# pycompression/python-zlib-ng

Measured on AMD Instinct MI355X. Metric: MB/s compress+decompress, 128 KiB blocks level 6, higher is better.
Workload: dtype u8

## Files before the change

### python-zlib-ng_amd/csrc/za_deflate.hip

```cpp
#include "za_common.h"
#include "za_crc.h"
#include <type_traits>

#define ZA_CH_GROUP 16
#define ZA_CH_OFFS(x) (((x) >> (32 - ZA_HASH_BITS - 2)) & (((1u << ZA_HASH_BITS) - 1u) << 2))
#define ZA_CH_CHUNK (64 * ZA_CH_GROUP)
#if defined(ZA_CH_STATS) || defined(ZA_ABL_CH_NOHASH) || defined(ZA_ABL_CH_NOATOMIC) || defined(ZA_ABL_CH_NOCHECK) || defined(ZA_ABL_CH_NOSTORE) || \
    defined(ZA_ABL_CH_HALFREADS) || defined(ZA_ABL_CH_HALFWRITES)
#undef ZA_CH_PAIR
#define ZA_CH_PAIR 0
#endif
#ifndef ZA_CH_PAIR
#define ZA_CH_PAIR 1
#endif
#ifdef ZA_CH_FORCE_FIX
#define ZA_CH_FORCE_FIX_ON true
#else
#define ZA_CH_FORCE_FIX_ON false
#endif

typedef uint32_t za_v4u32 __attribute__((ext_vector_type(4)));
__device__ __forceinline__ void za_issue_load16(za_v4u32 &dst, const uint8_t *addr)
{
    asm volatile("global_load_dwordx4 %0, %1, off" : "=v"(dst) : "v"(addr) : "memory");
// ... 893 lines not shown
            const uint32_t idx = P & (ZA_BYTES - 1), w = idx >> 2, sh = idx & 3u;
            const uint32_t m0 = win32[w], m1 = win32[w + 1], m2 = win32[w + 2], m3 = win32[w + 3], m4 = win32[w + 4];
            me0 = __builtin_amdgcn_alignbyte(m1, m0, sh); me1 = __builtin_amdgcn_alignbyte(m2, m1, sh);
            me2 = __builtin_amdgcn_alignbyte(m3, m2, sh); me3 = __builtin_amdgcn_alignbyte(m4, m3, sh);
        };
        auto finish = [&](int p, uint32_t P, uint32_t me0, uint32_t me1, uint32_t me2, uint32_t me3, int maxlen, int cap, int nice,
                          int best_len, int best_dist, uint32_t own_b, uint32_t own_c) {
#pragma unroll
            for (int t = 0; t < (USEC ? 2 : 1); t++) {
                const int dl = maxlen >= ZA_MIN_MATCH ? (int)(t == 0 ? own_b : own_c) : 0;
                if (dl != 0 && dl <= L.max_dist && best_len < nice) {
                    const uint32_t q = P - (uint32_t)dl;
                    const uint32_t sh = q & 3u;
                    const uint32_t *cw = (const uint32_t *)(lds + (q & (uint32_t)(ZA_BYTES - 4)));
                    const uint32_t c0 = cw[0], c1 = cw[1], c2 = cw[2], c3 = cw[3], c4 = cw[4];
                    const uint32_t x0 = __builtin_amdgcn_alignbyte(c1, c0, sh) ^ me0, x1 = __builtin_amdgcn_alignbyte(c2, c1, sh) ^ me1;
                    const uint32_t x2 = __builtin_amdgcn_alignbyte(c3, c2, sh) ^ me2, x3 = __builtin_amdgcn_alignbyte(c4, c3, sh) ^ me3;
                    uint32_t fbit, f1, f2, f3;
                    asm("v_ffbl_b32 %0, %4\n\tv_ffbl_b32 %1, %5\n\tv_ffbl_b32 %2, %6\n\tv_ffbl_b32 %3, %7\n\t"
                        "v_add_u32_e64 %1, %1, 32 clamp\n\tv_add_u32_e64 %2, %2, 64 clamp\n\tv_add_u32_e64 %3, %3, %8 clamp\n\t"
                        "v_min3_u32 %0, %0, %1, %2\n\tv_min_u32_e32 %0, %0, %3"
                        : "=&v"(fbit), "=&v"(f1), "=&v"(f2), "=&v"(f3) : "v"(x0), "v"(x1), "v"(x2), "v"(x3), "s"(96u));
                    int len = (int)min(fbit >> 3, 16u);
                    if (len == 16 && cap > 16) len = za_search_extend(win32, q, P, len, maxlen);
                    len = len < cap ? len : cap;
                    const bool better = len > best_len || (len == best_len && dl < best_dist);
                    best_len = better ? len : best_len;
                    best_dist = better ? dl : best_dist;
                }
            }
            uint32_t result = 0;
            if (best_len >= ZA_MIN_MATCH && !(best_len == 3 && best_dist > L.too_far3) && !(best_len == 4 && best_dist > L.too_far4))
                result = ((uint32_t)best_len << 15) | (uint32_t)(best_dist - 1);
            longm = longm || best_len > 64;
            best[p] = __builtin_amdgcn_perm(me0, result, 0x04020100u);
        };
        auto push = [&](bool alive, int p, uint32_t P, uint32_t q, int best_len, int best_dist, int depth) {
            const unsigned long long m = __ballot(alive);
            if (alive) {
                const uint32_t at = wl_n + __builtin_amdgcn_mbcnt_hi((uint32_t)(m >> 32), __builtin_amdgcn_mbcnt_lo((uint32_t)m, 0u));
                wl[2 * at] = (uint32_t)(p - base) | ((uint32_t)best_len << 12) | ((uint32_t)depth << 21);
                wl[2 * at + 1] = (P - q) | ((uint32_t)best_dist << 16);
            }
            wl_n += (uint32_t)__builtin_popcountll(m);
            __builtin_amdgcn_fence(__ATOMIC_RELEASE, "wavefront");
            __builtin_amdgcn_wave_barrier();
        };
        auto batch = [&](uint32_t nb) {
            wl_n -= nb;
            const bool has = (uint32_t)lane < nb;
            uint32_t e0 = 0, e1 = 0;
            __builtin_amdgcn_fence(__ATOMIC_ACQUIRE, "wavefront");
            if (has) { e0 = wl[2 * (wl_n + lane)]; e1 = wl[2 * (wl_n + lane) + 1]; }
            __builtin_amdgcn_fence(__ATOMIC_ACQ_REL, "wavefront");
            __builtin_amdgcn_wave_barrier();
            bool alive = false;
            int p = 0, best_len = 0, best_dist = 0, depth = 0;
            uint32_t P = 0, q = 0;
            if (has) {
                p = base + (int)(e0 & 0xFFFu);
                best_len = (int)((e0 >> 12) & 0x1FFu); depth = (int)(e0 >> 21); best_dist = (int)(e1 >> 16);
                P = goff + (uint32_t)(ZA_WIN + p);
                q = P - (e1 & 0xFFFFu);
                int seg_end = ((p >> sshift) + 1) << sshift;
                if (seg_end > n) seg_end = n;
                int maxlen = seg_end - p;
                if (maxlen > ZA_MAX_MATCH) maxlen = ZA_MAX_MATCH;
                const int cap = L.cap < maxlen ? L.cap : maxlen, nice = L.nice < cap ? L.nice : cap;
                uint32_t me0, me1, me2, me3;
                my16(P, me0, me1, me2, me3);
                const uint32_t sq = q % ZA_RING;
                uint32_t qb = RING_B0 + 2u * sq;
                uint32_t d = *(const uint16_t *)(lds + qb);
                alive = visit(P, me0, me1, me2, me3, maxlen, cap, nice, q, qb, d, best_len, best_dist, depth);
                if (!alive) finish(p, P, me0, me1, me2, me3, maxlen, cap, nice, best_len, best_dist, (uint32_t)linkb[p], USEC ? (uint32_t)linkc[p] : 0u);
            }
            push(alive, p, P, q, best_len, best_dist, depth);
        };
        uint32_t slot = (goff + (uint32_t)(ZA_WIN + base + tid)) % ZA_RING;
        load_own_links(base + ZA_SEARCH_TILE);
#pragma unroll
        for (int k = 0; k < ZA_SEARCH_TILE / ZA_SEARCH_THREADS; k++, slot = slot + ZA_SEARCH_THREADS >= ZA_RING ? slot + ZA_SEARCH_THREADS - ZA_RING : slot + ZA_SEARCH_THREADS) {
            const int p = base + k * ZA_SEARCH_THREADS + tid;
            bool alive = false;
            const uint32_t P = goff + (uint32_t)(ZA_WIN + p);
            uint32_t q = P;
            int best_len = ZA_MIN_MATCH - 1, best_dist = 0, depth = L.chain;
            if (p < n) {
                int seg_end = ((p >> sshift) + 1) << sshift;
                if (seg_end > n) seg_end = n;
                int maxlen = seg_end - p;
                if (maxlen > ZA_MAX_MATCH) maxlen = ZA_MAX_MATCH;
                uint32_t me0, me1, me2, me3;
                my16(P, me0, me1, me2, me3);
                const int cap = L.cap < maxlen ? L.cap : maxlen, nice = L.nice < cap ? L.nice : cap;
                if (maxlen >= ZA_MIN_MATCH) {
                    uint32_t qb = RING_B0 + 2u * slot;
                    uint32_t d = *(const uint16_t *)(lds + qb);
                    alive = visit(P, me0, me1, me2, me3, maxlen, cap, nice, q, qb, d, best_len, best_dist, depth);
                }
                if (!alive) finish(p, P, me0, me1, me2, me3, maxlen, cap, nice, best_len, best_dist, lkb[k], lkc[k]);
            }
            push(alive, p, P, q, best_len, best_dist, depth);
            while (__builtin_amdgcn_readfirstlane((int)wl_n) >= 64) batch(64u);
        }
        for (;;) {
            const uint32_t left = (uint32_t)__builtin_amdgcn_readfirstlane((int)wl_n);
            if (left == 0) break;
            batch(left < 64u ? left : 64u);
        }
        } else {
        uint32_t slot = (goff + (uint32_t)(ZA_WIN + base + (CONSEC ? 4 * tid : tid))) % ZA_RING;
        load_own_links(base + ZA_SEARCH_TILE);
        if (stats && base > 0) stats_issue(base - ZA_SEARCH_TILE);
#ifndef ZA_SEARCH_KUNROLL
#define ZA_SEARCH_KUNROLL 4
#endif
        const int p0c = base + 4 * tid;
        const uint32_t P0c = goff + (uint32_t)(ZA_WIN + p0c);
        uint32_t cm0 = 0, cm1 = 0, cm2 = 0, cm3 = 0, cm4 = 0;
        uint2 cdq = make_uint2(0u, 0u);
        int cseg_end = 0;
        if (CONSEC && p0c < n) {
            const uint32_t w = (P0c & (ZA_BYTES - 1)) >> 2;
            cm0 = win32[w]; cm1 = win32[w + 1]; cm2 = win32[w + 2]; cm3 = win32[w + 3]; cm4 = win32[w + 4];
            cdq = *(const uint2 *)(lds + RING_B0 + 2u * slot);
            cseg_end = ((p0c >> sshift) + 1) << sshift;
            if (cseg_end > n) cseg_end = n;
        }
#pragma unroll
        for (int k = 0; k < ZA_SEARCH_TILE / ZA_SEARCH_THREADS; k++, slot = CONSEC ? slot : slot + ZA_SEARCH_THREADS >= ZA_RING ? slot + ZA_SEARCH_THREADS - ZA_RING : slot + ZA_SEARCH_THREADS) {
            const int p = CONSEC ? p0c + k : base + k * ZA_SEARCH_THREADS + tid;
            res[k] = 0u;
            if (p >= n) continue;
            int seg_end = cseg_end;
            if (!CONSEC) {
                seg_end = ((p >> sshift) + 1) << sshift;
                if (seg_end > n) seg_end = n;
            }
            int maxlen = seg_end - p;
            if (maxlen > ZA_MAX_MATCH) maxlen = ZA_MAX_MATCH;
            uint32_t result = 0;
            const uint32_t P = goff + (uint32_t)(ZA_WIN + p);
            uint32_t me0, me1, me2, me3;
            if (CONSEC) {
                if (k == 0) { me0 = cm0; me1 = cm1; me2 = cm2; me3 = cm3; }
                else {
                    me0 = __builtin_amdgcn_alignbyte(cm1, cm0, (uint32_t)k); me1 = __builtin_amdgcn_alignbyte(cm2, cm1, (uint32_t)k);
                    me2 = __builtin_amdgcn_alignbyte(cm3, cm2, (uint32_t)k); me3 = __builtin_amdgcn_alignbyte(cm4, cm3, (uint32_t)k);
                }
            } else {
                const uint32_t idx = P & (ZA_BYTES - 1), w = idx >> 2, sh = idx & 3u;
                const uint32_t m0 = win32[w], m1 = win32[w + 1], m2 = win32[w + 2], m3 = win32[w + 3], m4 = win32[w + 4];
                me0 = __builtin_amdgcn_alignbyte(m1, m0, sh); me1 = __builtin_amdgcn_alignbyte(m2, m1, sh);
                me2 = __builtin_amdgcn_alignbyte(m3, m2, sh); me3 = __builtin_amdgcn_alignbyte(m4, m3, sh);
            }
            if (maxlen >= ZA_MIN_MATCH) {
                const int cap = L.cap < maxlen ? L.cap : maxlen;
                const int nice = L.nice < cap ? L.nice : cap;
                int best_len = ZA_MIN_MATCH - 1, best_dist = 0;
                uint32_t q = P;
                uint32_t qb = RING_B0 + 2u * (CONSEC ? slot + (uint32_t)k : slot);
                uint32_t d = CONSEC ? ((k < 2 ? cdq.x : cdq.y) >> (16 * (k & 1))) & 0xFFFFu : (uint32_t)*(const uint16_t *)(lds + qb);
                int depth = STEPS > 0 ? STEPS : L.chain;
#pragma unroll
                while (depth-- > 0) {
                    q -= d;
                    qb -= 2u * d;
                    qb += qb < RING_B0 ? RING_BYTES : 0u;
                    const int dist = (int)(P - q);
                    if (dist > L.max_dist) break;
                    d = *(const uint16_t *)(lds + qb);
                    const uint32_t sh = q & 3u;
                    const uint32_t *cw = (const uint32_t *)(lds + (q & (uint32_t)(ZA_BYTES - 4)));
                    const uint32_t c0 = cw[0], c1 = cw[1], c2 = cw[2], c3 = cw[3], c4 = cw[4];
                    uint32_t x0 = __builtin_amdgcn_alignbyte(c1, c0, sh) ^ me0;
                    uint32_t x1 = __builtin_amdgcn_alignbyte(c2, c1, sh) ^ me1;
                    uint32_t x2 = __builtin_amdgcn_alignbyte(c3, c2, sh) ^ me2;
                    uint32_t x3 = __builtin_amdgcn_alignbyte(c4, c3, sh) ^ me3;
                    uint32_t fbit, f1, f2, f3;
                    asm("v_ffbl_b32 %0, %4\n\tv_ffbl_b32 %1, %5\n\tv_ffbl_b32 %2, %6\n\tv_ffbl_b32 %3, %7\n\t"
                        "v_add_u32_e64 %1, %1, 32 clamp\n\tv_add_u32_e64 %2, %2, 64 clamp\n\tv_add_u32_e64 %3, %3, %8 clamp\n\t"
                        "v_min3_u32 %0, %0, %1, %2\n\tv_min_u32_e32 %0, %0, %3"
                        : "=&v"(fbit), "=&v"(f1), "=&v"(f2), "=&v"(f3) : "v"(x0), "v"(x1), "v"(x2), "v"(x3), "s"(96u));
                    int len = (int)min(fbit >> 3, FULL ? 16u : (uint32_t)cap);
                    if (FULL && len == 16 && cap > 16 && best_len < cap &&
                        (best_len < 16 || (uint8_t)za_lds_ld32(win32, q + (uint32_t)best_len) == (uint8_t)za_lds_ld32(win32, P + (uint32_t)best_len))) {
                        len = za_search_extend(win32, q, P, len, maxlen);
                    }
                    if (FULL) len = len < cap ? len : cap;
                    const bool better = len > best_len;
                    best_len = better ? len : best_len;
                    best_dist = better ? dist : best_dist;
                    if (best_len >= nice) break;
                }
                bool from_bc = false;
#ifndef ZA_ABL_SEARCH_NO_B
                {
                    const uint32_t dl = lkb[k];
#ifdef ZA_ABL_BC_SELF
                    const uint32_t q2 = P - (dl & 3u);
#else
                    const uint32_t q2 = P - dl;
#endif
                    const uint32_t *cw = (const uint32_t *)(lds + (q2 & (uint32_t)(ZA_BYTES - 4)));
                    const uint32_t c0 = cw[0], c1 = cw[1];
                    const uint32_t x = (__builtin_amdgcn_alignbyte(c1, c0, q2 & 3u) ^ me0) << 8;
                    const bool better = x == 0u && dl != 0u && (int)dl <= L.max_dist &&
                                        (ZA_HASH_BYTES_B > best_len || (ZA_HASH_BYTES_B == best_len && (int)dl < best_dist));
                    best_len = better ? ZA_HASH_BYTES_B : best_len;
                    best_dist = better ? (int)dl : best_dist;
                    from_bc = better;
                }
#endif
#ifndef ZA_ABL_SEARCH_NO_C
                if (USEC) {
                    const uint32_t dl = lkc[k];
#ifdef ZA_ABL_BC_SELF
                    const uint32_t q2 = P - (dl & 3u);
#else
                    const uint32_t q2 = P - dl;
#endif
                    const uint32_t sh = q2 & 3u;
                    const uint32_t *cw = (const uint32_t *)(lds + (q2 & (uint32_t)(ZA_BYTES - 4)));
                    const uint32_t c0 = cw[0], c1 = cw[1], c2 = cw[2], c3 = cw[3];
                    const uint32_t x = (__builtin_amdgcn_alignbyte(c1, c0, sh) ^ me0) | (__builtin_amdgcn_alignbyte(c2, c1, sh) ^ me1) |
                                       (__builtin_amdgcn_alignbyte(c3, c2, sh) ^ me2);
                    const bool better = x == 0u && dl != 0u && (int)dl <= L.max_dist && cap >= ZA_HASH_BYTES_C &&
                                        (ZA_HASH_BYTES_C > best_len || (ZA_HASH_BYTES_C == best_len && (int)dl < best_dist));
                    best_len = better ? ZA_HASH_BYTES_C : best_len;
                    best_dist = better ? (int)dl : best_dist;
                    from_bc = from_bc || better;
                }
#endif
#ifndef ZA_ABL_NO_EXTEND
                if (!FULL && (best_len == cap || from_bc) && best_len < maxlen) {
                    best_len = za_search_extend(win32, P - (uint32_t)best_dist, P, best_len, maxlen);
                }
#endif
                if (best_len >= ZA_MIN_MATCH && !(best_len == 3 && best_dist > L.too_far3) && !(best_len == 4 && best_dist > L.too_far4))
                    result = ((uint32_t)best_len << 15) | (uint32_t)(best_dist - 1);
                longm = longm || best_len > 64;
            }
#ifdef ZA_ABL_SEARCH_NOLIT
            res[k] = result;
#else
            res[k] = __builtin_amdgcn_perm(me0, result, 0x04020100u);
#endif
        }
        res_base = base;
        }
        if (pq < need_links) store_quad(pq, need_links, nq);
        {
            const int p = bytes_loaded + 8 * tid;
            if (p < need_bytes) {
                const uint64_t v = nbv >> nsh;
                store_bytes(p, (uint32_t)v);
                if (p + 4 < need_bytes) store_bytes(p + 4, (uint32_t)(v >> 32));
            }
        }
        if (ZA_OWN_STAGE) own_store(base + ZA_SEARCH_TILE);
        links_loaded = need_links; bytes_loaded = need_bytes;
        if (stats) { flush_results(); stats_use(); __syncthreads(); }
        else za_lds_barrier();
    }
    if constexpr (!FULL) flush_results();
    if (stats && n > 0) {
        __syncthreads();
        stats_issue((n - 1) & ~(ZA_SEARCH_TILE - 1));
        stats_use();
        for (int d = 32; d >= 1; d >>= 1) { st_U += (uint32_t)__shfl_xor((int)st_U, d, 64); st_NM += (uint32_t)__shfl_xor((int)st_NM, d, 64); }
        if ((tid & 63) == 0) { atomicAdd(&st_cnt[0], st_U); atomicAdd(&st_cnt[1], st_NM); }
        __syncthreads();
        const uint32_t U = st_cnt[0], NM = st_cnt[1];
        uint32_t hh = 0u;
        if (tid < 256) {
            hh = 16u * st_hist[tid] + 1u + (U >> 6);
            st_hist[tid] = 0u;
            uint32_t T = hh;
            for (int d = 32; d >= 1; d >>= 1) T += (uint32_t)__shfl_xor((int)T, d, 64);
            if ((tid & 63) == 0) atomicAdd(&st_cnt[2], T);
        }
        __syncthreads();
        if (tid < 256) {
            const uint32_t T = st_cnt[2];
            uint32_t *cost = cost_ws + (size_t)ui * ZA_DP_COSTS;
            int lbias = za_ilog4(U + NM, U ? U : 1u), mbias = za_ilog4(U + NM, NM ? NM : 1u);
            lbias = lbias > 24 ? 24 : lbias;
            mbias = mbias > 24 ? 24 : mbias;
            const int cl = za_ilog4(T, hh) + lbias;
            cost[tid] = (uint32_t)(cl < 12 ? 12 : cl > 52 ? 52 : cl);
            if (tid == 0) { cost[256] = (uint32_t)(12 + mbias + 20); cost[257] = 0u; }
        }
        __syncthreads();
        if (tid < 4) st_cnt[tid] = 0u;
        st_U = 0u; st_NM = 0u;
    }
    if (L.dp && __ballot(longm) != 0ull && (tid & 63) == 0) cost_ws[(size_t)ui * ZA_DP_COSTS + 258] = 1u;
    carry_bytes = bytes_loaded; n_prev = n;
    }
}

#define ZA_PCH 32
#define ZA_PROW (ZA_PCH + 1)
#ifndef ZA_DP_NEAR
#define ZA_DP_NEAR   64
#endif
#define ZA_DP_ROWS   (ZA_DP_NEAR / 2 + 4)
#ifndef ZA_DCH
#define ZA_DCH       16
#endif
#define ZA_DROW      (ZA_DCH + 1)
#define ZA_DPIECES   (ZA_DCH / 4)
#define ZA_DP_SEGSLOTS 2064

__global__ __launch_bounds__(256) void za_k_dpstats(const ZaUnit *__restrict__ units, const uint32_t *__restrict__ best_ws,
                                                    uint32_t *__restrict__ cost_ws )
{
    __shared__ uint32_t hist[256];
    __shared__ uint32_t cnt[3], tsum;
    const int n = (int)units[blockIdx.x].in_len;
    const int tid = (int)threadIdx.x, lane = tid & 63;
    const uint32_t *best = best_ws + (size_t)blockIdx.x * ZA_BEST_STRIDE;
    hist[tid] = 0;
    if (tid < 3) cnt[tid] = 0;
    if (tid == 0) tsum = 0;
    __syncthreads();
    uint32_t U = 0, NM = 0;
    for (int base = 1024 * (tid >> 6); base < n; base += 4096) {
        const int i0 = base + 4 * lane;
        uint4 v = make_uint4(0u, 0u, 0u, 0u);
        uint32_t pv = 0;
        if (i0 < n) v = *(const uint4 *)(best + i0);
        if (lane == 0 && i0 > 0 && i0 < n) pv = best[i0 - 1];
        const uint32_t e[4] = {v.x, v.y, v.z, v.w};
        uint32_t lp = (uint32_t)__shfl_up((int)ZA_ELEN(v.w), 1, 64);
        if (lane == 0) lp = ZA_ELEN(pv);
#pragma unroll
        for (int k = 0; k < 4; k++) {
            const uint32_t len = ZA_ELEN(e[k]);
            if (i0 + k < n) {
                if (len == 0u || (len == 3u && ZA_EDIST(e[k]) > (uint32_t)ZA_DP_WEAK_DIST)) { atomicAdd(&hist[e[k] >> 24], 1u); U++; }
                else if (len + 1u != lp) NM++;
            }
            lp = len;
        }
    }
    for (int d = 32; d >= 1; d >>= 1) { U += (uint32_t)__shfl_xor((int)U, d, 64); NM += (uint32_t)__shfl_xor((int)NM, d, 64); }
    if (lane == 0) { atomicAdd(&cnt[0], U); atomicAdd(&cnt[1], NM); }
    __syncthreads();
    U = cnt[0]; NM = cnt[1];
    const uint32_t hh = 16u * hist[tid] + 1u + (U >> 6);
    uint32_t T = hh;
    for (int d = 32; d >= 1; d >>= 1) T += (uint32_t)__shfl_xor((int)T, d, 64);
    if (lane == 0) atomicAdd(&tsum, T);
    __syncthreads();
    T = tsum;
    uint32_t *cost = cost_ws + (size_t)blockIdx.x * ZA_DP_COSTS;
    if (n == 0) return;
    int lbias = za_ilog4(U + NM, U ? U : 1u), mbias = za_ilog4(U + NM, NM ? NM : 1u);
    lbias = lbias > 24 ? 24 : lbias;
    mbias = mbias > 24 ? 24 : mbias;
    const int c = za_ilog4(T, hh) + lbias;
    cost[tid] = (uint32_t)(c < 12 ? 12 : c > 52 ? 52 : c);
    if (tid == 0) { cost[256] = (uint32_t)(12 + mbias + 20); cost[257] = 0u; }
}

__device__ __forceinline__ uint32_t za_pk_add_u16(uint32_t a, uint32_t b)
{
    uint32_t r;
    asm("v_pk_add_u16 %0, %1, %2" : "=v"(r) : "v"(a), "v"(b));
    return r;
}

__global__ __launch_bounds__(64) void za_k_optparse(const ZaUnit *__restrict__ units, uint32_t *__restrict__ best_ws,
                                                    const uint32_t *__restrict__ cost_ws, uint32_t *__restrict__ tok_ws ,
                                                    ZaLevel L)
{
    __shared__ uint32_t costt[ZA_DP_COSTS + 4];
    __shared__ uint32_t xt[3 * (ZA_MAX_MATCH + 1)];
    __shared__ uint32_t ring[ZA_DP_ROWS * 64];
    __shared__ uint32_t rowb[64 * ZA_DROW];
#ifndef ZA_DP_PAD
#define ZA_DP_PAD 2304
#endif
#if ZA_DP_PAD > 0
    __shared__ uint32_t dp_pad[ZA_DP_PAD / 4];
    if (units[blockIdx.x].in_len == 0xFFFFFFFFu) {
        dp_pad[threadIdx.x] = blockIdx.x; __syncthreads(); best_ws[threadIdx.x] = dp_pad[(threadIdx.x * 7u + best_ws[0]) % (ZA_DP_PAD / 4)];
    }
#endif
    const ZaUnit u = units[blockIdx.x];
    const int n = (int)u.in_len;
    const int lane = za_lane();
    const int sshift = ZA_UNIT_SEG_SHIFT(u.flags), seg = 1 << sshift;
    const int nseg = (n + seg - 1) >> sshift;
    uint32_t *best = best_ws + (size_t)blockIdx.x * ZA_BEST_STRIDE;
    if (n == 0) return;
    for (int i = lane; i < ZA_DP_COSTS; i += 64) costt[i] = cost_ws[(size_t)blockIdx.x * ZA_DP_COSTS + i];
    if (L.fixed_cost) {
        __syncthreads();
        for (int i = lane; i < 256; i += 64) costt[i] = i < 144 ? 32u : 36u;
        if (lane == 0) costt[256] = 48u;
    }
    for (int len = lane; len <= ZA_MAX_MATCH; len += 64) {
        const int l0 = len > 7 ? len - ZA_DP_SUB : 3;
        uint32_t x[ZA_DP_SUB + 1];
#pragma unroll
        for (int k = 0; k <= ZA_DP_SUB; k++) {
            const int l = l0 + k;
            int lc, ln = 0, le;
            if (l <= ZA_MAX_MATCH) za_len_sym(l, lc, ln, le);
            x[k] = (len >= 3 && l <= len && l >= L.min_len) ? (uint32_t)(4 * ln) : 0x3FFFu;
        }
        xt[3 * len] = x[0] | (x[1] << 16); xt[3 * len + 1] = x[2] | (x[3] << 16); xt[3 * len + 2] = x[4] | ((uint32_t)l0 << 16);
    }
    for (int i = lane; i < ZA_DP_ROWS * 64; i += 64) ring[i] = 0;
    __syncthreads();

    const int s0 = lane << sshift;
    int s1 = s0 + seg;
    if (s1 > n) s1 = n;
    const bool active = lane < nseg;
    uint32_t *myb = rowb + lane * ZA_DROW;
    uint8_t *myring = (uint8_t *)(ring + lane);
    uint16_t *accg = (uint16_t *)(tok_ws + (size_t)blockIdx.x * ZA_TOK_STRIDE) + (size_t)lane * ZA_DP_SEGSLOTS;
    auto ring_put = [&](int slot, uint32_t v) {
        *(uint16_t *)(myring + (slot >> 1) * 256 + (slot & 1) * 2) = (uint16_t)v;
        if (slot < 8) *(uint16_t *)(myring + ((slot >> 1) + ZA_DP_NEAR / 2) * 256 + (slot & 1) * 2) = (uint16_t)v;
    };
    const int mbase = (int)costt[256];
#ifdef ZA_ABL_DP_NOLONG
    const bool has_long = false;
#else
    const bool has_long = costt[258] != 0u;
#endif
    if (active) { ring_put((s1 - s0) & (ZA_DP_NEAR - 1), 0u); accg[s1 - s0] = 0; }
    int acc_next = 0;
    int far_base = -100;
    uint32_t fw[8] = {0u, 0u, 0u, 0u, 0u, 0u, 0u, 0u};
    uint4 pb[ZA_DPIECES];
    auto prefetch = [&](int c) {
#pragma unroll
        for (int j = 0; j < ZA_DPIECES; j++) {
            const int sg = (64 / ZA_DPIECES) * j + lane / ZA_DPIECES, off = (sg << sshift) + c * ZA_DCH + 4 * (lane % ZA_DPIECES);
            pb[j] = make_uint4(0, 0, 0, 0);
            if (c >= 0 && sg < nseg && off < n) pb[j] = *(const uint4 *)(best + off);
        }
    };
    struct Fetch { uint32_t e, clit, x0, x1, x2, w0, w1, w2; };
    auto stage_b = [&](uint32_t e, int idx_p) -> Fetch {
        Fetch f;
        f.e = e;
        f.clit = costt[e >> 24];
        const uint32_t len = ZA_ELEN(e);
        const uint32_t *xr = xt + 3u * len;
        f.x0 = xr[0]; f.x1 = xr[1]; f.x2 = xr[2];
        const uint32_t l0 = len > 7u ? len - (uint32_t)ZA_DP_SUB : 3u;
        const uint32_t st = ((uint32_t)idx_p + l0) & (uint32_t)(ZA_DP_NEAR - 1);
        const uint8_t *rp = myring + (st >> 1) * 256;
        f.w0 = *(const uint32_t *)rp; f.w1 = *(const uint32_t *)(rp + 256); f.w2 = *(const uint32_t *)(rp + 512);
        return f;
    };
    const int nch = ((n < seg ? n : seg) + ZA_DCH - 1) / ZA_DCH;
    uint4 po[ZA_DPIECES];
    uint32_t wacc[ZA_DCH / 2];
    int pend = -1;
    auto flush_pending = [&](auto longs_tag) {
        if (pend < 0) return;
        const int pcb = s0 + pend * ZA_DCH;
        if (decltype(longs_tag)::value && active && pcb < s1) {
            uint4 *g = (uint4 *)(accg + pend * ZA_DCH);
#pragma unroll
            for (int k = 0; k < ZA_DCH / 8; k++) g[k] = make_uint4(wacc[4 * k], wacc[4 * k + 1], wacc[4 * k + 2], wacc[4 * k + 3]);
        }
#pragma unroll
        for (int j = 0; j < ZA_DPIECES; j++) {
            const int sg = (64 / ZA_DPIECES) * j + lane / ZA_DPIECES, off = (sg << sshift) + pend * ZA_DCH + 4 * (lane % ZA_DPIECES);
            if (sg < nseg && off < n) *(uint4 *)(best + off) = po[j];
        }
    };
    prefetch(nch - 1);
    auto walk = [&](auto longs_tag) {
    constexpr bool LONGS = decltype(longs_tag)::value;
#pragma unroll 1
    for (int c = nch - 1; c >= 0; c--) {
        const int cb = s0 + c * ZA_DCH;
        __builtin_amdgcn_wave_barrier();
#pragma unroll
        for (int j = 0; j < ZA_DPIECES; j++) {
            uint32_t *r = rowb + ((64 / ZA_DPIECES) * j + lane / ZA_DPIECES) * ZA_DROW + 4 * (lane % ZA_DPIECES);
            r[0] = pb[j].x; r[1] = pb[j].y; r[2] = pb[j].z; r[3] = pb[j].w;
        }
        __builtin_amdgcn_fence(__ATOMIC_RELEASE, "wavefront");
        __builtin_amdgcn_wave_barrier();
        __builtin_amdgcn_fence(__ATOMIC_ACQUIRE, "wavefront");
        flush_pending(longs_tag);
        prefetch(c - 1);
        if (__ballot(active && cb < s1) != 0ull) {
            const int ib = c * ZA_DCH;
            uint32_t e_a = myb[ZA_DCH - 2];
            Fetch f = stage_b(myb[ZA_DCH - 1], ib + ZA_DCH - 1);
#pragma unroll 4
            for (int j = ZA_DCH - 1; j >= 0; j--) {
                const int idx = ib + j;
                const bool live = active && cb + j < s1;
                const Fetch g = f;
                if (j >= 1) f = stage_b(e_a, idx - 1);
                if (j >= 2) e_a = myb[j - 2];
                const uint32_t e = g.e, len = ZA_ELEN(e), dm1 = e & 0x7FFFu, l0 = g.x2 >> 16;
                const uint32_t st1 = ((uint32_t)idx + l0) & 1u;
                uint32_t v0 = __builtin_amdgcn_alignbyte(g.w1, g.w0, 2u * st1), v1 = __builtin_amdgcn_alignbyte(g.w2, g.w1, 2u * st1);
                uint32_t v2 = st1 ? g.w2 >> 16 : g.w2;
                if (LONGS && __builtin_expect(__ballot(live && len > (uint32_t)ZA_DP_NEAR) != 0ull, 0)) {
                    if (live && len > (uint32_t)ZA_DP_NEAR) {
                        const int e_lo = idx + (int)len - ZA_DP_SUB;
                        if (e_lo < far_base || e_lo + ZA_DP_SUB > far_base + 15) {
                            far_base = (e_lo + ZA_DP_SUB - 14) & ~1;
                            __builtin_amdgcn_fence(__ATOMIC_ACQ_REL, "workgroup");
                            const uint32_t *g32 = (const uint32_t *)(accg + far_base);
#pragma unroll
                            for (int k = 0; k < 8; k++) fw[k] = __hip_atomic_load(g32 + k, __ATOMIC_RELAXED, __HIP_MEMORY_SCOPE_AGENT);
                        }
                        const uint32_t o = (uint32_t)(e_lo - far_base), q = o >> 1;
                        uint32_t w0 = fw[0], w1 = fw[1], w2 = fw[2];
#pragma unroll
                        for (uint32_t k = 1; k <= 5; k++) { w0 = q == k ? fw[k] : w0; w1 = q == k ? fw[k + 1] : w1; w2 = q == k ? fw[k + 2] : w2; }
                        const uint32_t sh = (o & 1u) * 2u;
                        v0 = __builtin_amdgcn_alignbyte(w1, w0, sh); v1 = __builtin_amdgcn_alignbyte(w2, w1, sh);
                        v2 = (o & 1u) ? w2 >> 16 : w2;
                    }
                }
                int de = 30 - (int)__builtin_clz(dm1 | 1u);
                de = de < 0 ? 0 : de;
                const uint32_t b16 = (uint32_t)(mbase + 4 * de - acc_next) & 0xFFFFu;
                const uint32_t bb = b16 | (b16 << 16);
                uint32_t sA = za_pk_add_u16(za_pk_add_u16(v0, g.x0), bb);
                const uint32_t sB = za_pk_add_u16(za_pk_add_u16(v1, g.x1), bb);
                const uint32_t sC = za_pk_add_u16(za_pk_add_u16(v2, g.x2), bb);
                if (l0 == 3u && dm1 >= (uint32_t)L.too_far3) sA = (sA & 0xFFFF0000u) | 0x3FFFu;
#ifdef ZA_DP_TAGS_SHIFT
                const int t0 = (__builtin_amdgcn_sbfe((int)sA, 0, 16) << 3) | 4, t1 = (((int)sA >> 16) << 3) | 3;
                const int t2 = (__builtin_amdgcn_sbfe((int)sB, 0, 16) << 3) | 2, t3 = (((int)sB >> 16) << 3) | 1;
                const int t4 = __builtin_amdgcn_sbfe((int)sC, 0, 16) << 3;
#else
                int t0, t1, t2, t3, t4;
                asm("v_mad_i32_i16 %0, %5, 8, 4\n\tv_mad_i32_i16 %1, %5, 8, 3 op_sel:[1,0,0,0]\n\t"
                    "v_mad_i32_i16 %2, %6, 8, 2\n\tv_mad_i32_i16 %3, %6, 8, 1 op_sel:[1,0,0,0]\n\tv_mad_i32_i16 %4, %7, 8, 0"
                    : "=&v"(t0), "=&v"(t1), "=&v"(t2), "=&v"(t3), "=&v"(t4) : "v"(sA), "v"(sB), "v"(sC));
#endif
                int t = t0 < t1 ? t0 : t1;
                t = t < t2 ? t : t2;
                int tb = t3 < t4 ? t3 : t4;
                t = t < tb ? t : tb;
                const int mc = t >> 3;
                const bool ok = mc < (int)g.clit;
                const int c_best = ok ? mc : (int)g.clit;
                const uint32_t choice = ok ? l0 + 4u - ((uint32_t)t & 7u) : 0u;
                if (live) {
                    acc_next += c_best;
                    ring_put(idx & (ZA_DP_NEAR - 1), (uint32_t)acc_next);
                    myb[j] = (e & (ok ? 0xFF007FFFu : 0xFF000000u)) | (choice << 15);
                }
            }
        }
        __builtin_amdgcn_fence(__ATOMIC_RELEASE, "wavefront");
        __builtin_amdgcn_wave_barrier();
        __builtin_amdgcn_fence(__ATOMIC_ACQUIRE, "wavefront");
        if (LONGS && active && cb < s1) {
            const uint8_t *rp = myring + ((c * ZA_DCH) & (ZA_DP_NEAR - 1)) / 2 * 256;
#pragma unroll
            for (int k = 0; k < ZA_DCH / 2; k++) wacc[k] = *(const uint32_t *)(rp + 256 * k);
        }
#pragma unroll
        for (int j = 0; j < ZA_DPIECES; j++) {
            const uint32_t *r = rowb + ((64 / ZA_DPIECES) * j + lane / ZA_DPIECES) * ZA_DROW + 4 * (lane % ZA_DPIECES);
            po[j] = make_uint4(r[0], r[1], r[2], r[3]);
        }
        pend = c;
    }
    flush_pending(longs_tag);
    };
    if (has_long) walk(std::true_type{}); else walk(std::false_type{});
}

template <bool FILT> __device__ __forceinline__ uint32_t za_minlen(uint32_t lf, const ZaLevel &L)
{
    return (!FILT || lf >= (uint32_t)L.min_len) ? lf : 0u;
}



template <bool FILT>
__global__ __launch_bounds__(64) void za_k_parse(const ZaUnit *__restrict__ units,
                                                 const uint32_t *__restrict__ best_ws, uint32_t *__restrict__ tok_ws,
                                                 uint32_t *__restrict__ segtok_ws, uint32_t *__restrict__ hist_ws,
                                                 uint32_t *__restrict__ crc_out,
                                                 const uint32_t *__restrict__ crc_table,
                                                 const uint32_t *__restrict__ x8k_table,
                                                 ZaLevel L)
{
    __shared__ uint32_t hist[ZA_HIST_STRIDE];
    __shared__ uint32_t crct[256];
    __shared__ uint32_t rowb[64 * ZA_PROW + 3];
    const ZaUnit u = units[blockIdx.x];
    const int n = (int)u.in_len;
    const int lane = za_lane();
    const int sshift = ZA_UNIT_SEG_SHIFT(u.flags), seg = 1 << sshift;
    const int nseg = (n + seg - 1) >> sshift;
    for (int i = lane; i < ZA_HIST_STRIDE; i += 64) hist[i] = 0;
    for (int i = lane; i < 256; i += 64) crct[i] = crc_table[i];
    __syncthreads();

    const int s0 = lane << sshift;
    int s1 = s0 + seg;
    if (s1 > n) s1 = n;
    const bool active = lane < nseg;
    const uint32_t *best = best_ws + (size_t)blockIdx.x * ZA_BEST_STRIDE;
    uint32_t *myb = rowb + lane * ZA_PROW;

    uint4 pb[8];
    auto prefetch = [&](int c) {
        const int rel = c * ZA_PCH;
#pragma unroll
        for (int j = 0; j < 8; j++) {
            const int sg = 8 * j + (lane >> 3), off = (sg << sshift) + rel;
            pb[j] = make_uint4(0, 0, 0, 0);
            if (c < seg / ZA_PCH && sg < nseg && off < n) {
                typedef uint32_t za_v4u __attribute__((ext_vector_type(4)));
                const za_v4u v = __builtin_nontemporal_load((const za_v4u *)(best + off + 4 * (lane & 7)));
                pb[j] = make_uint4(v.x, v.y, v.z, v.w);
            }
        }
    };

    uint32_t ntok = 0;
    uint32_t crc_r = 0xFFFFFFFFu;
    int p = s0;
    uint32_t carry_b = 0;
    uint32_t nchunk = 0;
    prefetch(0);
#pragma unroll 1
    for (int c = 0; c < seg / ZA_PCH; c++) {
        const int cb = s0 + c * ZA_PCH;
        if (__ballot(active && cb < s1) == 0ull) break;
        __builtin_amdgcn_wave_barrier();
#pragma unroll
        for (int j = 0; j < 8; j++) {
            uint32_t *r = rowb + (8 * j + (lane >> 3)) * ZA_PROW + 1 + 4 * (lane & 7);
            r[0] = pb[j].x; r[1] = pb[j].y; r[2] = pb[j].z; r[3] = pb[j].w;
        }
        myb[0] = carry_b;
        __builtin_amdgcn_wave_barrier();
        prefetch(c + 1);
        int ce = cb + ZA_PCH;
        if (ce > s1) ce = s1;
        if (active && cb < s1) {
#ifndef ZA_ABL_PARSE_NOCRC
            {
                int k = cb;
                for (; k + 4 <= ce; k += 4) {
                    const uint32_t *e = myb + 1 + (k - cb);
                    const uint32_t w4 = __builtin_amdgcn_perm(e[1], e[0], 0x0c0c0703u) | __builtin_amdgcn_perm(e[3], e[2], 0x07030c0cu);
                    crc_r = crct[(crc_r ^ w4) & 0xFF] ^ (crc_r >> 8);
                    crc_r = crct[(crc_r ^ (w4 >> 8)) & 0xFF] ^ (crc_r >> 8);
                    crc_r = crct[(crc_r ^ (w4 >> 16)) & 0xFF] ^ (crc_r >> 8);
                    crc_r = crct[(crc_r ^ (w4 >> 24)) & 0xFF] ^ (crc_r >> 8);
                }
                for (; k < ce; k++) crc_r = crct[(crc_r ^ (myb[1 + k - cb] >> 24)) & 0xFF] ^ (crc_r >> 8);
            }
#endif
            {
                const int lim = ce == s1 ? ce : ce - 1;
                auto push = [&](uint32_t t) {
                    myb[nchunk] = t;
                    nchunk++;
                };
                while (p < lim) {
                    const uint32_t b = myb[p - cb + 1], bn = myb[p - cb + 2], e2 = myb[p - cb + 3];
                    const uint32_t lf = za_minlen<FILT>(ZA_ELEN(b), L), nlf = za_minlen<FILT>(ZA_ELEN(bn), L);
                    const bool is_match = lf != 0u;
                    const int len = (int)lf;
                    const uint32_t lit = b >> 24;
                    const int dist = is_match ? (int)ZA_EDIST(b) : 1;
                    int lc, ln, le, dc, dn, de;
                    za_len_sym(is_match ? len : 3, lc, ln, le);
                    za_dist_sym(dist, dc, dn, de);
                    const bool c1 = lf == 0u && p + 1 < ce && nlf == 0u;
                    const bool c2 = c1 && p + 2 < ce && za_minlen<FILT>(ZA_ELEN(e2), L) == 0u;
                    const uint32_t l1 = bn >> 24, l2 = e2 >> 24;
                    const uint32_t t = is_match ? (0x80000000u | ((uint32_t)lc << 26) | ((uint32_t)le << 21) | ((uint32_t)dc << 16) | (uint32_t)de)
                                                : lit | (c1 ? l1 << 8 : 0u) | (c2 ? l2 << 16 : 0u) | (((c1 ? 1u : 0u) + (c2 ? 1u : 0u)) << 24);
                    push(t);
#ifndef ZA_ABL_PARSE_NOHIST
                    atomicAdd(&hist[is_match ? 257u + (uint32_t)lc : lit], 1u);
                    if (is_match) atomicAdd(&hist[288 + dc], 1u);
                    if (c1) atomicAdd(&hist[l1], 1u);
                    if (c2) atomicAdd(&hist[l2], 1u);
#endif
                    p += is_match ? len : 1 + (c1 ? 1 : 0) + (c2 ? 1 : 0);
                }
            }
            carry_b = myb[ZA_PCH];
        }
        __builtin_amdgcn_fence(__ATOMIC_RELEASE, "wavefront");
        __builtin_amdgcn_wave_barrier();
#pragma unroll
        for (int j = 0; j < 8; j++) {
            const int sg = 8 * j + (lane >> 3);
            const uint32_t cnt = (uint32_t)__shfl((int)nchunk, sg, 64), at = (uint32_t)__shfl((int)ntok, sg, 64);
            const uint32_t first = 4u * (uint32_t)(lane & 7);
            const uint32_t *r = rowb + sg * ZA_PROW;
            uint32_t *dst = tok_ws + (size_t)blockIdx.x * ZA_TOK_STRIDE + ((size_t)sg << sshift) + at;
            if (first < cnt) {
                if (at + first + 4u <= (uint32_t)seg) { ZaU4u v; v.x = r[first]; v.y = r[first + 1]; v.z = r[first + 2]; v.w = r[first + 3]; *(ZaU4u *)(dst + first) = v; }
                else for (uint32_t i = first; i < cnt && i < first + 4u; i++) dst[i] = r[i];
            }
            if ((lane & 7) == 7 && cnt > 32u) dst[32] = r[32];
        }
        ntok += nchunk; nchunk = 0;
        __builtin_amdgcn_wave_barrier();
    }
    uint32_t cseg = 0;
    if (active) {
        cseg = crc_r ^ 0xFFFFFFFFu;
        if (lane < nseg - 1) {
            const int tail = n - ((nseg - 1) << sshift);
            uint32_t xt = 0x80000000u, sq = 0x00800000u;
            for (int m = tail; m; m >>= 1) { if (m & 1) xt = za_multmodp(sq, xt); sq = za_multmodp(sq, sq); }
            uint32_t xk = 0x80000000u;
            if (sshift == ZA_SEG_SHIFT) xk = x8k_table[nseg - 2 - lane];
            else {
                uint32_t xs = 0x00800000u;
                for (int i = 0; i < sshift; i++) xs = za_multmodp(xs, xs);
                for (int m = nseg - 2 - lane; m; m >>= 1) { if (m & 1) xk = za_multmodp(xs, xk); xs = za_multmodp(xs, xs); }
            }
            cseg = za_multmodp(za_multmodp(xk, xt), cseg);
        }
    }
    cseg = za_wave_xor_reduce(cseg);
    if (lane == 0) crc_out[blockIdx.x] = cseg;
    segtok_ws[(size_t)blockIdx.x * ZA_MAX_SEGS + lane] = ntok;
    __syncthreads();
    if (lane == 0) hist[256] = 1;
    __syncthreads();
    for (int i = lane; i < ZA_HIST_STRIDE; i += 64) hist_ws[(size_t)blockIdx.x * ZA_HIST_STRIDE + i] = hist[i];
}

#define ZA_RCH 64
#define ZA_RROW (ZA_RCH / 4 + 1)
#define ZA_RTOK 68
#define ZA_RTROW (ZA_RTOK + 1)
template <bool RUNS>
__global__ __launch_bounds__(64) void za_k_parse_rle(const uint8_t *__restrict__ in, const ZaUnit *__restrict__ units,
                                                     uint32_t *__restrict__ tok_ws, uint32_t *__restrict__ segtok_ws,
                                                     uint32_t *__restrict__ hist_ws, uint32_t *__restrict__ crc_out,
                                                     const uint32_t *__restrict__ crc_table,
                                                     const uint32_t *__restrict__ x8k_table)
{
    __shared__ uint32_t hist[ZA_HIST_STRIDE];
    __shared__ uint32_t crct[256];
    __shared__ uint32_t rowb[64 * ZA_RROW];
    __shared__ uint32_t tokb[64 * ZA_RTROW];
    const ZaUnit u = units[blockIdx.x];
    const int n = (int)u.in_len;
    const int lane = za_lane();
    const int sshift = ZA_UNIT_SEG_SHIFT(u.flags), seg = 1 << sshift;
    const int nseg = (n + seg - 1) >> sshift;
    for (int i = lane; i < ZA_HIST_STRIDE; i += 64) hist[i] = 0;
    for (int i = lane; i < 256; i += 64) crct[i] = crc_table[i];
    __syncthreads();

    const uint8_t *ub = in + u.in_off;
    const int s0 = lane << sshift;
    int s1 = s0 + seg;
    if (s1 > n) s1 = n;
    const bool active = lane < nseg;
    const int sh = (int)((uintptr_t)(ub + s0) & 15u);
    const int rend = active ? sh + (s1 - s0) : 0;
    const uint32_t *myrow = rowb + lane * ZA_RROW;
    uint32_t *mytok = tokb + lane * ZA_RTROW;

    typedef uint32_t za_v4u __attribute__((ext_vector_type(4)));
    za_v4u pb[4];
    auto prefetch = [&](int c) {
#pragma unroll
        for (int j = 0; j < 4; j++) {
            const int sg = 16 * j + (lane >> 2);
            pb[j] = za_v4u{0u, 0u, 0u, 0u};
            if (sg < nseg) {
                const uint8_t *first = ub + (sg << sshift);
                const int send = ((sg + 1) << sshift) < n ? ((sg + 1) << sshift) : n;
                const uint8_t *a = (const uint8_t *)((uintptr_t)first & ~(uintptr_t)15) + c * ZA_RCH + 16 * (lane & 3);
                if (a < ub + send) pb[j] = __builtin_nontemporal_load((const za_v4u *)a);
            }
        }
    };

    uint32_t crc_r = 0xFFFFFFFFu;
    uint32_t ntok = 0, nchunk = 0;
    uint32_t litw = 0, litn = 0;
    uint32_t prev = 0x100u, pend = 0;
    if (RUNS && active && (s0 > 0 || u.dict_len > 0)) prev = ub[s0 - 1];
    bool done = !active;
    auto push = [&](uint32_t t) { mytok[nchunk] = t; nchunk++; };
    auto lit = [&](uint32_t b) {
        litw |= b << (8u * litn);
        atomicAdd(&hist[b], 1u);
        if (++litn == 3u) { push(litw | (2u << 24)); litw = 0; litn = 0; }
    };
    auto flush_lits = [&]() { if (litn) { push(litw | ((litn - 1u) << 24)); litw = 0; litn = 0; } };
    auto match = [&](uint32_t len) {
        flush_lits();
        int lc, ln, le;
        za_len_sym((int)len, lc, ln, le);
        push(0x80000000u | ((uint32_t)lc << 26) | ((uint32_t)le << 21));
        atomicAdd(&hist[257 + lc], 1u);
        atomicAdd(&hist[288], 1u);
    };
    auto close_run = [&]() {
        if (pend >= 3u) match(pend);
        else for (uint32_t k = 0; k < pend; k++) lit(prev);
        pend = 0;
    };

    const int nch = (15 + (n < seg ? n : seg) + ZA_RCH - 1) / ZA_RCH;
    prefetch(0);
#pragma unroll 1
    for (int c = 0; c < nch; c++) {
        const int ib = c * ZA_RCH;
        if (__ballot(ib < rend) == 0ull) break;
        __builtin_amdgcn_wave_barrier();
#pragma unroll
        for (int j = 0; j < 4; j++) {
            uint32_t *r = rowb + (16 * j + (lane >> 2)) * ZA_RROW + 4 * (lane & 3);
            r[0] = pb[j].x; r[1] = pb[j].y; r[2] = pb[j].z; r[3] = pb[j].w;
        }
        __builtin_amdgcn_wave_barrier();
        prefetch(c + 1);
        if (ib < rend) {
#pragma unroll 2
            for (int k = 0; k < ZA_RCH / 4; k++) {
                const uint32_t w = myrow[k];
#pragma unroll
                for (int b = 0; b < 4; b++) {
                    const int i = ib + 4 * k + b;
                    if (i >= sh && i < rend) {
                        const uint32_t x = (w >> (8 * b)) & 0xFFu;
                        crc_r = crct[(crc_r ^ x) & 0xFFu] ^ (crc_r >> 8);
                        if (RUNS && x == prev) {
                            if (++pend == (uint32_t)ZA_MAX_MATCH) { match(pend); pend = 0; }
                        } else {
                            if (RUNS) { close_run(); prev = x; }
                            lit(x);
                        }
                    }
                }
            }
        }
        if (!done && rend <= ib + ZA_RCH) {
            if (RUNS) close_run();
            flush_lits();
            done = true;
        }
        __builtin_amdgcn_fence(__ATOMIC_RELEASE, "wavefront");
        __builtin_amdgcn_wave_barrier();
#pragma unroll
        for (int j = 0; j < 8; j++) {
            const int sg = 8 * j + (lane >> 3);
            const uint32_t cnt = (uint32_t)__shfl((int)nchunk, sg, 64), at = (uint32_t)__shfl((int)ntok, sg, 64);
            const uint32_t *r = tokb + sg * ZA_RTROW;
            uint32_t *dst = tok_ws + (size_t)blockIdx.x * ZA_TOK_STRIDE + ((size_t)sg << sshift) + at;
#pragma unroll
            for (int q = 0; q < 3; q++) {
                const uint32_t first = 4u * (uint32_t)((lane & 7) + 8 * q);
                if (first < cnt) {
                    if (at + first + 4u <= (uint32_t)seg) { ZaU4u v; v.x = r[first]; v.y = r[first + 1]; v.z = r[first + 2]; v.w = r[first + 3]; *(ZaU4u *)(dst + first) = v; }
                    else for (uint32_t i = first; i < cnt && i < first + 4u; i++) dst[i] = r[i];
                }
            }
        }
        ntok += nchunk; nchunk = 0;
        __builtin_amdgcn_wave_barrier();
    }
    uint32_t cseg = 0;
    if (active) {
        cseg = crc_r ^ 0xFFFFFFFFu;
        if (lane < nseg - 1) {
            const int tail = n - ((nseg - 1) << sshift);
            uint32_t xt = 0x80000000u, sq = 0x00800000u;
            for (int m = tail; m; m >>= 1) { if (m & 1) xt = za_multmodp(sq, xt); sq = za_multmodp(sq, sq); }
            uint32_t xk = 0x80000000u;
            if (sshift == ZA_SEG_SHIFT) xk = x8k_table[nseg - 2 - lane];
            else {
                uint32_t xs = 0x00800000u;
                for (int i = 0; i < sshift; i++) xs = za_multmodp(xs, xs);
                for (int m = nseg - 2 - lane; m; m >>= 1) { if (m & 1) xk = za_multmodp(xs, xk); xs = za_multmodp(xs, xs); }
            }
            cseg = za_multmodp(za_multmodp(xk, xt), cseg);
        }
    }
    cseg = za_wave_xor_reduce(cseg);
    if (lane == 0) crc_out[blockIdx.x] = cseg;
    segtok_ws[(size_t)blockIdx.x * ZA_MAX_SEGS + lane] = ntok;
    __syncthreads();
    if (lane == 0) hist[256] = 1;
    __syncthreads();
    for (int i = lane; i < ZA_HIST_STRIDE; i += 64) hist_ws[(size_t)blockIdx.x * ZA_HIST_STRIDE + i] = hist[i];
}

__global__ __launch_bounds__(64) void za_k_unit_crc(const uint8_t *__restrict__ in, const ZaUnit *__restrict__ units,
                                                    uint32_t *__restrict__ crc_out, const uint32_t *__restrict__ crc_table,
                                                    const uint32_t *__restrict__ x8k_table)
{
    __shared__ uint32_t crct[256];
    const ZaUnit u = units[blockIdx.x];
    for (int i = za_lane(); i < 256; i += 64) crct[i] = crc_table[i];
    __syncthreads();
    const uint32_t c = za_wave_crc32(in + u.in_off, (int)u.in_len, crct, x8k_table);
    if (za_lane() == 0) crc_out[blockIdx.x] = c;
}

struct ZaPlanLds {
    uint32_t key[288];
    __attribute__((aligned(16))) uint32_t A[288];
    uint32_t freq[320];
    uint8_t lens[320];
    uint16_t codes[320];
    uint8_t seq[320];
    uint16_t cltok[320];
    uint32_t clf[19];
    uint8_t cl_lens[19];
    uint16_t cl_codes[19];
    int m;
    int btype;
};

__device__ void za_sort_syms(ZaPlanLds &S, const uint32_t *freq, int nsym)
{
    const int lane = za_lane();
    __syncthreads();
    int m = 0;
    for (int base = 0; base < nsym; base += 64) {
        const int i = base + lane;
        const uint32_t k = (i < nsym && freq[i]) ? ((freq[i] << 9) | (uint32_t)i) : 0u;
        const unsigned long long nz = __ballot(k != 0u);
        if (k) S.A[m + (int)__builtin_amdgcn_mbcnt_hi((uint32_t)(nz >> 32), __builtin_amdgcn_mbcnt_lo((uint32_t)nz, 0u))] = k;
        m += (int)__builtin_popcountll(nz);
    }
    __syncthreads();
    for (int idx = lane; idx < m; idx += 64) {
        const uint32_t k = S.A[idx];
        int rank = 0;
        int j = 0;
        for (; j + 4 <= m; j += 4) {
            const uint4 o = *(const uint4 *)&S.A[j];
            rank += (o.x < k) + (o.y < k) + (o.z < k) + (o.w < k);
        }
        for (; j < m; j++) rank += S.A[j] < k;
        S.key[rank] = k;
    }
    __syncthreads();
    if (lane == 0) S.m = m;
    __syncthreads();
}

__device__ void za_lengths_wave(ZaPlanLds &S, int nsym, int limit, uint8_t *lens)
{
    const int lane = za_lane();
    __syncthreads();
    const int m = S.m;
    for (int i = lane; i < nsym; i += 64) lens[i] = 0;
    __syncthreads();
    if (m == 0) return;
    if (m == 1) { if (lane == 0) lens[S.key[0] & 511u] = 1; __syncthreads(); return; }
    uint32_t *A = S.A;
    uint16_t *dep = S.cltok;
    for (int i = lane; i < m; i += 64) A[i] = S.key[i] >> 9;
    __syncthreads();
    if (lane == 0) {
        const uint32_t NONE = 0xFFFFFFFFu;
        const uint32_t a0 = A[0] + A[1];
        A[0] = a0;
        int root = 0, leaf = 2;
        uint32_t wr = a0;
        uint32_t fl = leaf < m ? A[leaf] : NONE, fl1 = leaf + 1 < m ? A[leaf + 1] : NONE;
        for (int next = 1; next < m - 1; next++) {
            uint32_t w;
            if (fl == NONE || wr < fl) { w = wr; A[root] = (uint32_t)next; root++; wr = root < next ? A[root] : NONE; }
            else { w = fl; leaf++; fl = fl1; fl1 = leaf + 1 < m ? A[leaf + 1] : NONE; }
            if (fl == NONE || (root < next && wr < fl)) { w += wr; A[root] = (uint32_t)next; root++; wr = root < next ? A[root] : NONE; }
            else { w += fl; leaf++; fl = fl1; fl1 = leaf + 1 < m ? A[leaf + 1] : NONE; }
            A[next] = w;
            if (root == next) wr = w;
        }
    }
    __syncthreads();
    const int ninner = m - 1, top = m - 2;
    int pi[5], di[5];
#pragma unroll
    for (int k = 0; k < 5; k++) {
        const int i = lane + 64 * k;
        pi[k] = top; di[k] = 0;
        if (i < top) { pi[k] = (int)A[i]; di[k] = 1; }
    }
    __syncthreads();
#pragma unroll
    for (int k = 0; k < 5; k++) { const int i = lane + 64 * k; if (i < ninner) { A[i] = (uint32_t)pi[k]; dep[i] = (uint16_t)di[k]; } }
    for (int round = 0; round < 10; round++) {
        __syncthreads();
        int np[5], nd[5];
        bool open = false;
#pragma unroll
        for (int k = 0; k < 5; k++) {
            const int i = lane + 64 * k;
            np[k] = pi[k]; nd[k] = di[k];
            if (i < ninner) { np[k] = (int)A[pi[k]]; nd[k] = di[k] + (int)dep[pi[k]]; open = open || np[k] != top; }
        }
        __syncthreads();
#pragma unroll
        for (int k = 0; k < 5; k++) {
            const int i = lane + 64 * k;
            pi[k] = np[k]; di[k] = nd[k];
// ... 631 lines not shown
```

Measured before the change: 59820.

## Align parse token stores to 32-byte sectors by staging a carried token tail

The parse kernel now keeps an aligned token staging area in front of each lane's LDS row. Each chunk flushes only a multiple of 8 (or 16) tokens to global memory, and the unflushed remainder is carried to the start of the row for the next chunk. The final chunk is rounded up. The aim is to replace scalar and unaligned partial writes with full aligned vector stores that cover whole memory sectors. In exchange it adds an LDS copy of the leftover tail each chunk, a possible second store pass, and larger shared rows, and the rounded-up final flush writes padding tokens past the real count.

After: 59860, median of 2. No clear change (+0.1%).

```diff
diff --git a/python-zlib-ng_amd/csrc/za_deflate.hip b/python-zlib-ng_amd/csrc/za_deflate.hip
--- a/python-zlib-ng_amd/csrc/za_deflate.hip
+++ b/python-zlib-ng_amd/csrc/za_deflate.hip
@@ -1219,7 +1219,10 @@
 }
 
 #define ZA_PCH 32
-#define ZA_PROW (ZA_PCH + 1)
+#ifndef ZA_PTOK_ALIGN
+#define ZA_PTOK_ALIGN 8
+#endif
+#define ZA_PROW (ZA_PTOK_ALIGN + ZA_PCH + 1)
 #ifndef ZA_DP_NEAR
 #define ZA_DP_NEAR   64
 #endif
@@ -1519,7 +1522,8 @@
 {
     __shared__ uint32_t hist[ZA_HIST_STRIDE];
     __shared__ uint32_t crct[256];
-    __shared__ uint32_t rowb[64 * ZA_PROW + 3];
+    __shared__ uint32_t rowb[64 * ZA_PROW + ZA_PTOK_ALIGN];
+    static_assert(ZA_PTOK_ALIGN == 8 || ZA_PTOK_ALIGN == 16, "a tail of one or two 32-byte sectors");
     const ZaUnit u = units[blockIdx.x];
     const int n = (int)u.in_len;
     const int lane = za_lane();
@@ -1534,7 +1538,8 @@
     if (s1 > n) s1 = n;
     const bool active = lane < nseg;
     const uint32_t *best = best_ws + (size_t)blockIdx.x * ZA_BEST_STRIDE;
-    uint32_t *myb = rowb + lane * ZA_PROW;
+    uint32_t *myt = rowb + lane * ZA_PROW;
+    uint32_t *myb = myt + ZA_PTOK_ALIGN;
 
     uint4 pb[8];
     auto prefetch = [&](int c) {
@@ -1555,7 +1560,7 @@
     uint32_t crc_r = 0xFFFFFFFFu;
     int p = s0;
     uint32_t carry_b = 0;
-    uint32_t nchunk = 0;
+    uint32_t nrow = 0;
     prefetch(0);
 #pragma unroll 1
     for (int c = 0; c < seg / ZA_PCH; c++) {
@@ -1564,7 +1569,7 @@
         __builtin_amdgcn_wave_barrier();
 #pragma unroll
         for (int j = 0; j < 8; j++) {
-            uint32_t *r = rowb + (8 * j + (lane >> 3)) * ZA_PROW + 1 + 4 * (lane & 7);
+            uint32_t *r = rowb + (8 * j + (lane >> 3)) * ZA_PROW + ZA_PTOK_ALIGN + 1 + 4 * (lane & 7);
             r[0] = pb[j].x; r[1] = pb[j].y; r[2] = pb[j].z; r[3] = pb[j].w;
         }
         myb[0] = carry_b;
@@ -1590,8 +1595,8 @@
             {
                 const int lim = ce == s1 ? ce : ce - 1;
                 auto push = [&](uint32_t t) {
-                    myb[nchunk] = t;
-                    nchunk++;
+                    myt[nrow] = t;
+                    nrow++;
                 };
                 while (p < lim) {
                     const uint32_t b = myb[p - cb + 1], bn = myb[p - cb + 2], e2 = myb[p - cb + 3];
@@ -1620,22 +1625,39 @@
             }
             carry_b = myb[ZA_PCH];
         }
+        const bool last = active && cb < s1 && ce == s1;
+        const uint32_t nst = (nrow + (last ? (uint32_t)ZA_PTOK_ALIGN - 1u : 0u)) & ~((uint32_t)ZA_PTOK_ALIGN - 1u);
         __builtin_amdgcn_fence(__ATOMIC_RELEASE, "wavefront");
         __builtin_amdgcn_wave_barrier();
+        uint32_t *tok_unit = tok_ws + (size_t)blockIdx.x * ZA_TOK_STRIDE;
 #pragma unroll
         for (int j = 0; j < 8; j++) {
             const int sg = 8 * j + (lane >> 3);
-            const uint32_t cnt = (uint32_t)__shfl((int)nchunk, sg, 64), at = (uint32_t)__shfl((int)ntok, sg, 64);
+            const uint32_t cnt = (uint32_t)__shfl((int)nst, sg, 64), at = (uint32_t)__shfl((int)ntok, sg, 64);
             const uint32_t first = 4u * (uint32_t)(lane & 7);
-            const uint32_t *r = rowb + sg * ZA_PROW;
-            uint32_t *dst = tok_ws + (size_t)blockIdx.x * ZA_TOK_STRIDE + ((size_t)sg << sshift) + at;
-            if (first < cnt) {
-                if (at + first + 4u <= (uint32_t)seg) { ZaU4u v; v.x = r[first]; v.y = r[first + 1]; v.z = r[first + 2]; v.w = r[first + 3]; *(ZaU4u *)(dst + first) = v; }
-                else for (uint32_t i = first; i < cnt && i < first + 4u; i++) dst[i] = r[i];
-            }
-            if ((lane & 7) == 7 && cnt > 32u) dst[32] = r[32];
-        }
-        ntok += nchunk; nchunk = 0;
+            const uint32_t *r = rowb + sg * ZA_PROW + first;
+            if (first < cnt) *(uint4 *)(tok_unit + ((size_t)sg << sshift) + at + first) = make_uint4(r[0], r[1], r[2], r[3]);
+        }
+        if (__ballot(nst > 32u) != 0ull) {
+#pragma unroll 1
+            for (int j = 0; j < 8; j++) {
+                const int sg = 8 * j + (lane >> 3);
+                const uint32_t cnt = (uint32_t)__shfl((int)nst, sg, 64), at = (uint32_t)__shfl((int)ntok, sg, 64);
+                const uint32_t first = 32u + 4u * (uint32_t)(lane & 7);
+                const uint32_t *r = rowb + sg * ZA_PROW + first;
+                if (first < cnt) *(uint4 *)(tok_unit + ((size_t)sg << sshift) + at + first) = make_uint4(r[0], r[1], r[2], r[3]);
+            }
+        }
+        __builtin_amdgcn_wave_barrier();
+        if (nst != 0u && !last) {
+            uint32_t t[ZA_PTOK_ALIGN];
+#pragma unroll
+            for (int i = 0; i < ZA_PTOK_ALIGN; i++) t[i] = myt[nst + i];
+#pragma unroll
+            for (int i = 0; i < ZA_PTOK_ALIGN; i++) myt[i] = t[i];
+        }
+        ntok += last ? nrow : nst;
+        nrow = last ? 0u : nrow - nst;
         __builtin_amdgcn_wave_barrier();
     }
     uint32_t cseg = 0;
```
